# wwyuan2023/VITS

Hardware: AMD Instinct MI355X
Metric: 22.05 kHz audio samples/sec/GPU (infer RTF) + train utt/sec at 1/2/4/8 MI355X (higher is better)
Workload: dtype fp32; 1 GPU; SynthesizerTrn.infer_p2 batch=16 Tx=100 Ty=500 (configs/base.json, 16 kHz, hop 192) per GPU; global_batch=16, seq_len=500, parallelism=single GPU, graph=False

## Files before the change

### vits_amd/csrc/resblock_f32p.hip

```cpp
#include <type_traits>

#include "conv1d_impl.h"

namespace {

using vits_conv::fast_sigmoid;
using vits_conv::fast_tanh;
using vits_conv::split3_bf16x4;

constexpr int RP_GROUP = 3;
struct RpGroup {
  vits_resblock_pair_desc d[RP_GROUP];
  int n;
  int batch;
  int bn;
};

typedef __bf16 bf16x8 __attribute__((ext_vector_type(8)));
typedef __bf16 bf16x4 __attribute__((ext_vector_type(4)));
typedef __bf16 bf16x2 __attribute__((ext_vector_type(2)));
typedef float f32x4v __attribute__((ext_vector_type(4)));

template <int MODE>
struct RpT {
  typedef float xt;
  typedef __bf16 lt;
  static constexpr int NPL = 3;
};
template <>
struct RpT<1> {
  typedef __bf16 xt;
  typedef __bf16 lt;
  static constexpr int NPL = 1;
};
template <>
struct RpT<2> {
  typedef _Float16 xt;
  typedef _Float16 lt;
  static constexpr int NPL = 1;
};
__host__ __device__ constexpr int rp_npl(int mode) { return mode == 0 ? 3 : 1; }

__host__ __device__ constexpr int rp_ng(int C) { return C <= 64 ? 256 : 128; }
#ifndef VITS_RP_TM64
#define VITS_RP_TM64 1
#endif
#ifndef VITS_RP_TM128
#define VITS_RP_TM128 1
#endif
#ifndef VITS_RP_TM256
#define VITS_RP_TM256 1
#endif
#ifdef VITS_RP_OTHER_SIDE
#define VITS_RP_SIDE(tm) (3 - (tm))
#else
#define VITS_RP_SIDE(tm) (tm)
#endif
__host__ __device__ constexpr int rp_tm(int C, int mode = 0) {
  return C == 32     ? 1
         : mode != 0 ? 2
         : C == 64   ? VITS_RP_SIDE(VITS_RP_TM64)
         : C == 128  ? VITS_RP_SIDE(VITS_RP_TM128)
                     : VITS_RP_SIDE(VITS_RP_TM256);
}
__host__ __device__ constexpr int rp_threads(int C, int tm) {
  return (C / (32 * tm)) * (rp_ng(C) / 64) * 64;
}
#ifndef VITS_RP_KC32
#define VITS_RP_KC32 32
#endif
__host__ __device__ constexpr int rp_kc(int C, int mode = 0) {
  return C == 256 ? 64 : C == 32 ? VITS_RP_KC32 : 16;
}
__host__ __device__ inline int rp_xcols(int NG, int k, int dil) {
  return ((NG + (k - 1) * dil + 3 + 3) >> 2) << 2;
}
__host__ __device__ inline int rp_lds_bytes(int C, int k, int dil, int mode = 0) {
  const int NG = rp_ng(C), npl = rp_npl(mode);
  const int nbuf = rp_kc(C, mode) < C ? 2 : 1;
  const int xs = nbuf * npl * rp_xcols(NG, k, dil) * (rp_kc(C, mode) + 4);
  const int gsz = npl * (NG + 16) * (C / 2 + 8);
  return 4 * 2 * C + 2 * (xs > gsz ? xs : gsz) + 64;
}
__host__ __device__ constexpr int rp_occ(int C, int, int tm) {
  return tm == 1 && C >= 64 ? 4 : C == 256 ? 1 : 2;
}

__device__ __forceinline__ float rp_gate(float a, float b) {
#pragma clang fp contract(off)
  return fast_tanh(a) * fast_sigmoid(b);
}

__device__ __forceinline__ float rp_max(float a, float b) {
  float r;
  asm("v_max_f32 %0, %1, %2" : "=v"(r) : "v"(a), "v"(b));
  return r;
}

template <typename T>
__device__ __forceinline__ T rp_fresh(T v) {
  asm volatile("" : "+v"(v));
  return v;
}

template <typename T>
__device__ __forceinline__ const T* rp_sbase(const T* p) {
  uint64_t u = reinterpret_cast<uint64_t>(p);
  asm("" : "+s"(u));
  return (const T*)reinterpret_cast<const __attribute__((address_space(1))) T*>(u);
}

template <int C, int MODE = 0, bool MEAN = false, int TM = rp_tm(C, MODE)>
__global__ __launch_bounds__(rp_threads(C, TM), rp_occ(C, MODE, TM)) void resblock_f32p_kernel(
    const RpGroup G) {
  typedef std::integral_constant<bool, true> edge_t;
  typedef std::integral_constant<bool, false> interior_t;
  typedef typename RpT<MODE>::xt xt;
  typedef typename RpT<MODE>::lt lt;
  constexpr int NPL = RpT<MODE>::NPL;
  typedef lt lt8 __attribute__((ext_vector_type(8)));
  typedef lt lt4 __attribute__((ext_vector_type(4)));
  typedef lt lt2 __attribute__((ext_vector_type(2)));
  typedef xt xt4 __attribute__((ext_vector_type(4)));
  constexpr int H = C / 2;
  static_assert(TM == 1 || (TM == 2 && C >= 64), "wave tile rows");
  constexpr int NT = rp_threads(C, TM);
  constexpr int WAVES_M = C / (32 * TM);
  constexpr int WAVES_N = NT / 64 / WAVES_M;
  constexpr int NG = 64 * WAVES_N;
  static_assert(NG == rp_ng(C), "tile columns");
  constexpr int TN = 2;
  constexpr int KC = rp_kc(C, MODE);
  constexpr int KCP = KC + 4;
  constexpr int GP = H + 8;
  constexpr int GPL = (NG + 16) * GP;
  constexpr int S1 = C / 16, S2 = H / 16;
  constexpr int NU = ((KC / 4) * ((NG + 102) / 4) + NT - 1) / NT;
  typedef lt8 av_t;
  constexpr int NB = NPL == 3 ? TN : 1;
  constexpr bool REMAT = TM == 1 && C >= 64;

  const int gi = MEAN ? 0 : (int)blockIdx.z / G.batch;
  const int b = (int)blockIdx.z - gi * G.batch;
  const int Tn = G.d[gi].t_len;
  const int L = G.d[gi].lengths ? min(Tn, (int)G.d[gi].lengths[b]) : Tn;
  const int BN = MEAN ? G.bn : NG - (G.d[gi].k - 1);
  const int n0 = blockIdx.x * BN;
  if (n0 >= Tn) return;
  if (G.d[gi].lengths && G.d[gi].len_skip > 0 && n0 >= L + G.d[gi].len_skip) return;

  extern __shared__ float smem[];
  float* const erow = smem;
  lt* const reg = reinterpret_cast<lt*>(smem + 2 * C);

  const int tid = threadIdx.x;
  const int lane = tid & 63;
  const int wid = __builtin_amdgcn_readfirstlane(tid >> 6);
  const int wn = (wid % WAVES_N) * 64;
  const int wm = (wid / WAVES_N) * (32 * TM);
  const int l32 = lane & 31;
  const int lhi = lane >> 5;

  float msum[TM][TN][MEAN ? 16 : 1];

#pragma unroll 1
  for (int br = 0; br < (MEAN ? G.n : 1); ++br) {
    const vits_resblock_pair_desc& p = G.d[MEAN ? br : gi];
    const int k = p.k;
    const int dil = p.dil;
    const int p1 = (k - 1) * dil / 2;
    const int p2 = (k - 1) / 2;
    const int tw0 = n0 - p2 - p1;
    const int xstart = tw0 & ~3;
    const int xcols = rp_xcols(NG, k, dil);
    const bool interior = xstart >= 0 && xstart + xcols <= Tn && n0 - p2 + NG <= L;
    if (MEAN && br > 0) __syncthreads();

    {
      const float* cond = p.cond ? p.cond + (int64_t)b * p.cond_bstride : nullptr;
      for (int r = tid; r < 2 * C; r += NT) {
        float e = 0.f;
        if (r < C) {
          const int idx = (r & 1) ? H + (r >> 1) : (r >> 1);
          if (p.b1) e = p.b1[idx];
          if (cond) e += cond[idx];
        } else if (p.b2) {
          e = p.b2[r - C];
        }
        erow[r] = e;
      }
    }

    f32x16 acc[TM][TN];
#pragma unroll
    for (int i = 0; i < TM; ++i)
#pragma unroll
      for (int j = 0; j < TN; ++j)
#pragma unroll
        for (int r = 0; r < 16; ++r) acc[i][j][r] = 0.f;

    auto mma = [&](av_t (*a)[TM], const av_t* bh, const av_t* bm, const av_t* bl) {
#pragma unroll
      for (int mi = 0; mi < TM; ++mi)
#pragma unroll
        for (int ni = 0; ni < TN; ++ni) {
          f32x16 c = acc[mi][ni];
          if constexpr (MODE == 0) {
            c = __builtin_amdgcn_mfma_f32_32x32x16_bf16(a[0][mi], bl[ni], c, 0, 0, 0);
            c = __builtin_amdgcn_mfma_f32_32x32x16_bf16(a[2][mi], bh[ni], c, 0, 0, 0);
            c = __builtin_amdgcn_mfma_f32_32x32x16_bf16(a[1][mi], bm[ni], c, 0, 0, 0);
            c = __builtin_amdgcn_mfma_f32_32x32x16_bf16(a[0][mi], bm[ni], c, 0, 0, 0);
            c = __builtin_amdgcn_mfma_f32_32x32x16_bf16(a[1][mi], bh[ni], c, 0, 0, 0);
            c = __builtin_amdgcn_mfma_f32_32x32x16_bf16(a[0][mi], bh[ni], c, 0, 0, 0);
          } else if constexpr (MODE == 1) {
            c = __builtin_amdgcn_mfma_f32_32x32x16_bf16(a[0][mi], bh[ni], c, 0, 0, 0);
          } else {
            c = __builtin_amdgcn_mfma_f32_32x32x16_f16(a[0][mi], bh[ni], c, 0, 0, 0);
          }
          acc[mi][ni] = c;
        }
    };
    auto loadA = [&](const lt* w, uint32_t al, int64_t wstep, int m_pad, int s, int total,
                     av_t (*a)[TM]) {
      const lt* wp = w + (int64_t)(s < total ? s : total - 1) * wstep + (int64_t)wm * 8;
      const uint32_t av = REMAT ? rp_fresh(al) : al;
#pragma unroll
      for (int q = 0; q < NPL; ++q)
#pragma unroll
        for (int mi = 0; mi < TM; ++mi)
          if constexpr (REMAT)
            a[q][mi] = *reinterpret_cast<const av_t*>(
                reinterpret_cast<const char*>(rp_sbase(wp + ((int64_t)q * m_pad + mi * 32) * 8)) +
                av);
          else
            a[q][mi] = *reinterpret_cast<const av_t*>(
                reinterpret_cast<const char*>(wp + ((int64_t)q * m_pad + mi * 32) * 8) + av);
    };

    av_t a0[NPL][TM], a1[NPL][TM];
    av_t bh0[TN], bm0[NB], bl0[NB], bh1[TN], bm1[NB], bl1[NB];

    const xt* xb = reinterpret_cast<const xt*>(p.x) + (int64_t)b * p.x_bstride;
    {
      const int xsh = tw0 - xstart;
      const int nunits = (KC / 4) * (xcols >> 2);
      const int xpl = xcols * KCP;
      lt* const xbuf0 = reg;
      lt* const xbuf1 = reg + NPL * xpl;
      const float slope = p.in_slope;
      constexpr bool XB = KC * sizeof(xt) <= 2 * C;
      constexpr uint32_t XU = XB ? (uint32_t)sizeof(xt) : 1u;
      xt4 xr[NU][4];
      uint32_t xoff[NU];
      bool xok[NU];
#pragma unroll
      for (int q = 0; q < NU; ++q) {
        const int u = tid + NT * q;
        const int tt = xstart + 4 * (u / (KC / 4));
        xok[q] = u < nunits && tt >= 0 && tt < Tn;
        xoff[q] = xok[q] ? (uint32_t)(4 * (u % (KC / 4)) * p.x_cstride + tt) * XU : 0;
      }
      auto gload = [&](int ch) __attribute__((always_inline)) {
        const xt* base = xb + (int64_t)ch * KC * p.x_cstride;
#pragma unroll
        for (int q = 0; q < NU; ++q) {
          if (q * NT < nunits) {
            const uint32_t xo = REMAT ? rp_fresh(xoff[q]) : xoff[q];
#pragma unroll
            for (int i = 0; i < 4; ++i) {
              const xt* row = base + (int64_t)i * p.x_cstride;
              if constexpr (REMAT) row = rp_sbase(row);
              xr[q][i] = *reinterpret_cast<const xt4*>(reinterpret_cast<const char*>(row) +
                                                       (size_t)xo * (sizeof(xt) / XU));
            }
          }
        }
      };
      const bool xfast = interior && slope > 0.f && slope < 1.f;
      auto lstore_as = [&](lt* xs, auto edge) __attribute__((always_inline)) {
        const int ftid = REMAT ? rp_fresh(tid) : tid;
#pragma unroll
        for (int q = 0; q < NU; ++q) {
          const int u = ftid + NT * q;
          if (q * NT < nunits && u < nunits) {
            f32x4v v[4];
#pragma unroll
            for (int i = 0; i < 4; ++i)
#pragma unroll
              for (int e = 0; e < 4; ++e) {
                float t = (float)xr[q][i][e];
                if constexpr (decltype(edge)::value) {
                  t = t < 0.f ? t * slope : t;
                  v[i][e] = xok[q] ? t : 0.f;
                } else {
                  v[i][e] = rp_max(t, t * slope);
                }
              }
            lt* xh = xs + 4 * (u / (KC / 4)) * KCP + 4 * (u % (KC / 4));
#pragma unroll
            for (int e = 0; e < 4; ++e) {
              const f32x4v w = {v[0][e], v[1][e], v[2][e], v[3][e]};
              if constexpr (NPL == 3) {
                bf16x4 h4, m4, l4;
                split3_bf16x4(w, h4, m4, l4);
                *reinterpret_cast<bf16x4*>(xh + e * KCP) = h4;
                *reinterpret_cast<bf16x4*>(xh + xpl + e * KCP) = m4;
                *reinterpret_cast<bf16x4*>(xh + 2 * xpl + e * KCP) = l4;
              } else {
                lt4 w4;
#pragma unroll
                for (int i = 0; i < 4; ++i) w4[i] = (lt)w[i];
                *reinterpret_cast<lt4*>(xh + e * KCP) = w4;
              }
            }
          }
        }
      };
      auto lstore = [&](lt* xs) __attribute__((always_inline)) {
        if (xfast)
          lstore_as(xs, interior_t());
        else
          lstore_as(xs, edge_t());
      };
      auto loadB = [&](const lt* xs, int j, int g, av_t* bh, av_t* bm, av_t* bl) {
        const int P4 = xpl / 4;
#pragma unroll
        for (int ni = 0; ni < TN; ++ni) {
          const lt4* xp = reinterpret_cast<const lt4*>(
              xs + (wn + ni * 32 + l32 + j * dil + xsh) * KCP + 16 * g + 8 * lhi);
          bh[ni] = __builtin_shufflevector(xp[0], xp[1], 0, 1, 2, 3, 4, 5, 6, 7);
          if constexpr (NPL == 3) {
            bm[ni] = __builtin_shufflevector(xp[P4], xp[P4 + 1], 0, 1, 2, 3, 4, 5, 6, 7);
            bl[ni] = __builtin_shufflevector(xp[2 * P4], xp[2 * P4 + 1], 0, 1, 2, 3, 4, 5, 6, 7);
          }
        }
      };
      const lt* wl = reinterpret_cast<const lt*>(p.w1);
      const uint32_t al = (uint32_t)((lhi * NPL) * p.m_pad1 + l32) * (uint32_t)(8 * sizeof(lt));
      const int64_t wstep = (int64_t)16 * NPL * p.m_pad1;
      const int total = S1 * k;
      const int nst = (KC / 16) * k;
      loadA(wl, al, wstep, p.m_pad1, 0, total, a0);
      gload(0);
      lstore(xbuf0);
      __syncthreads();
      for (int ch = 0; ch < C / KC; ++ch) {
        const bool more = ch + 1 < C / KC;
        if (more) gload(ch + 1);
        const lt* xs = (ch & 1) ? xbuf1 : xbuf0;
        const int s0 = ch * nst;
        int j = 0, g = 0;
        auto next = [&]() {
          if (++j == k) {
            j = 0;
            ++g;
          }
        };
        loadB(xs, 0, 0, bh0, bm0, bl0);
        int st = 0;
        for (; st + 2 <= nst; st += 2) {
          next();
          loadA(wl, al, wstep, p.m_pad1, s0 + st + 1, total, a1);
          loadB(xs, j, g, bh1, bm1, bl1);
          __builtin_amdgcn_sched_barrier(0);
          mma(a0, bh0, bm0, bl0);
          __builtin_amdgcn_sched_barrier(0);
          next();
          loadA(wl, al, wstep, p.m_pad1, s0 + st + 2, total, a0);
          if (st + 2 < nst) loadB(xs, j, g, bh0, bm0, bl0);
          __builtin_amdgcn_sched_barrier(0);
          mma(a1, bh1, bm1, bl1);
          __builtin_amdgcn_sched_barrier(0);
        }
        if (st < nst) {
          loadA(wl, al, wstep, p.m_pad1, s0 + nst, total, a1);
          __builtin_amdgcn_sched_barrier(0);
          mma(a0, bh0, bm0, bl0);
#pragma unroll
          for (int q = 0; q < NPL; ++q)
#pragma unroll
            for (int mi = 0; mi < TM; ++mi) a0[q][mi] = a1[q][mi];
        }
        if (more) lstore((ch & 1) ? xbuf0 : xbuf1);
        __syncthreads();
      }
    }

    lt* const gs = reg;
    auto gate = [&](auto edge) __attribute__((always_inline)) {
      const int flane = REMAT ? rp_fresh(lane) : lane;
      const int l32 = flane & 31, lhi = flane >> 5;
#pragma unroll
      for (int mi = 0; mi < TM; ++mi) {
        f32x4v er[4];
#pragma unroll
        for (int g = 0; g < 4; ++g)
          er[g] = *reinterpret_cast<const f32x4v*>(erow + wm + mi * 32 + 4 * lhi + 8 * g);
#pragma unroll
        for (int ni = 0; ni < TN; ++ni) {
          const int col = wn + ni * 32 + l32;
          const int t = n0 - p2 + col;
          const bool in = t >= 0 && t < L;
#pragma unroll
          for (int r = 0; r < 16; r += 4) {
            const int row = wm + mi * 32 + 4 * lhi + 8 * (r >> 2);
            const f32x4v e = er[r >> 2];
            float g0 = rp_gate(acc[mi][ni][r] + e[0], acc[mi][ni][r + 1] + e[1]);
            float g1 = rp_gate(acc[mi][ni][r + 2] + e[2], acc[mi][ni][r + 3] + e[3]);
            if constexpr (decltype(edge)::value) {
              g0 = in ? g0 : 0.f;
              g1 = in ? g1 : 0.f;
            }
            lt* gp = gs + col * GP + (row >> 1);
            if constexpr (NPL == 3) {
              const f32x4v w = {g0, g1, 0.f, 0.f};
              bf16x4 h4, m4, l4;
              split3_bf16x4(w, h4, m4, l4);
              *reinterpret_cast<bf16x2*>(gp) = __builtin_shufflevector(h4, h4, 0, 1);
              *reinterpret_cast<bf16x2*>(gp + GPL) = __builtin_shufflevector(m4, m4, 0, 1);
              *reinterpret_cast<bf16x2*>(gp + 2 * GPL) = __builtin_shufflevector(l4, l4, 0, 1);
            } else {
              lt2 v2;
              v2[0] = (lt)g0;
              v2[1] = (lt)g1;
              *reinterpret_cast<lt2*>(gp) = v2;
            }
          }
#pragma unroll
          for (int r = 0; r < 16; ++r) acc[mi][ni][r] = 0.f;
        }
      }
    };
    if (interior)
      gate(interior_t());
    else
      gate(edge_t());
    for (int i = tid; i < NPL * 16 * H; i += NT) {
      const int pl = i / (16 * H);
      const int e = i - pl * 16 * H;
      gs[pl * GPL + (NG + e / H) * GP + e % H] = (lt)0.f;
    }
    __syncthreads();

    {
      const int flane = REMAT ? rp_fresh(lane) : lane;
      const int l32 = flane & 31, lhi = flane >> 5;
      const lt* wl = reinterpret_cast<const lt*>(p.w2);
      const uint32_t al = (uint32_t)((lhi * NPL) * p.m_pad2 + l32) * (uint32_t)(8 * sizeof(lt));
      const int64_t wstep = (int64_t)16 * NPL * p.m_pad2;
      const int total = S2 * k;
      const lt* gl = gs + (wn + l32) * GP + 8 * lhi;
      int j = 0, g = 0;
      auto loadB = [&](av_t* bh, av_t* bm, av_t* bl) {
        const lt* x = gl + j * GP + 16 * g;
#pragma unroll
        for (int ni = 0; ni < TN; ++ni) {
          bh[ni] = *reinterpret_cast<const av_t*>(x + ni * 32 * GP);
          if constexpr (NPL == 3) {
            bm[ni] = *reinterpret_cast<const av_t*>(x + ni * 32 * GP + GPL);
            bl[ni] = *reinterpret_cast<const av_t*>(x + ni * 32 * GP + 2 * GPL);
          }
        }
        if (++j == k) {
          j = 0;
          ++g;
        }
      };
      loadA(wl, al, wstep, p.m_pad2, 0, total, a0);
      loadB(bh0, bm0, bl0);
      int s = 0;
      for (; s + 2 <= total; s += 2) {
        loadA(wl, al, wstep, p.m_pad2, s + 1, total, a1);
        loadB(bh1, bm1, bl1);
        __builtin_amdgcn_sched_barrier(0);
        mma(a0, bh0, bm0, bl0);
        __builtin_amdgcn_sched_barrier(0);
        loadA(wl, al, wstep, p.m_pad2, s + 2, total, a0);
        if (s + 2 < total) loadB(bh0, bm0, bl0);
        __builtin_amdgcn_sched_barrier(0);
        mma(a1, bh1, bm1, bl1);
        __builtin_amdgcn_sched_barrier(0);
      }
      if (s < total) mma(a0, bh0, bm0, bl0);
    }

    xt* const yb = reinterpret_cast<xt*>(p.y) + (int64_t)b * p.y_bstride;
    const bool accum = !MEAN && p.accumulate;
    const float div = MEAN ? (float)G.n : p.post_div;
    const bool last = !MEAN || br == G.n - 1;
    auto epilogue = [&](auto edge) __attribute__((always_inline)) {
      const int flane = REMAT ? rp_fresh(lane) : lane;
      const int l32 = flane & 31, lhi = flane >> 5;
#pragma unroll
      for (int mi = 0; mi < TM; ++mi) {
        const xt* const xrow = xb + (int64_t)(wm + mi * 32) * p.x_cstride;
        xt* const yrow = yb + (int64_t)(wm + mi * 32) * p.y_cstride;
        f32x4v e2[4];
#pragma unroll
        for (int g = 0; g < 4; ++g)
          e2[g] = *reinterpret_cast<const f32x4v*>(erow + C + wm + mi * 32 + 4 * lhi + 8 * g);
#pragma unroll
        for (int ni = 0; ni < TN; ++ni) {
          const int col = wn + ni * 32 + l32;
          const int t = n0 + col;
          const bool st = decltype(edge)::value ? col < BN && t < Tn : col < BN;
          const int tc = st ? t : 0;
          const uint32_t xv = (uint32_t)(4 * lhi * p.x_cstride + tc) * (uint32_t)sizeof(xt);
          const uint32_t yv = (uint32_t)(4 * lhi * p.y_cstride + tc) * (uint32_t)sizeof(xt);
          auto xat = [&](int r) __attribute__((always_inline)) -> const xt& {
            const xt* row = xrow + (int64_t)((r & 3) + 8 * (r >> 2)) * p.x_cstride;
            return *reinterpret_cast<const xt*>(reinterpret_cast<const char*>(row) + xv);
          };
          auto yat = [&](int r) __attribute__((always_inline)) -> xt& {
            xt* row = yrow + (int64_t)((r & 3) + 8 * (r >> 2)) * p.y_cstride;
            return *reinterpret_cast<xt*>(reinterpret_cast<char*>(row) + yv);
          };
          float o[16];
#pragma unroll
          for (int r = 0; r < 16; ++r) {
            const float rv = (float)xat(r);
            const float v = acc[mi][ni][r] + e2[r >> 2][r & 3];
            o[r] = rv + v;
          }
          if constexpr (MEAN) {
#pragma unroll
            for (int r = 0; r < 16; ++r) {
              o[r] = br == 0 ? o[r] : msum[mi][ni][r] + o[r];
              msum[mi][ni][r] = o[r];
            }
          }
          if (accum) {
#pragma unroll
            for (int r = 0; r < 16; ++r)
              o[r] = (float)yat(r) + o[r];
          }
          if (last) {
            if (div != 1.0f) {
#pragma unroll
              for (int r = 0; r < 16; ++r) o[r] = o[r] / div;
            }
            if (st) {
#pragma unroll
              for (int r = 0; r < 16; ++r) {
                if constexpr (decltype(edge)::value) o[r] = t < L ? o[r] : 0.f;
                yat(r) = (xt)o[r];
              }
            }
          }
        }
      }
    };
    if (interior)
      epilogue(interior_t());
    else
      epilogue(edge_t());
  }
}

template <int C, int MODE = 0, bool MEAN = false, int TM = rp_tm(C, MODE)>
int rp_launch(const RpGroup& g, hipStream_t s) {
  int lds = 0, gx = 0;
  for (int i = 0; i < g.n; ++i) {
    const vits_resblock_pair_desc& d = g.d[i];
    const int l = rp_lds_bytes(C, d.k, d.dil, MODE);
    if (l > lds) lds = l;
    const int BN = MEAN ? g.bn : rp_ng(C) - (d.k - 1);
    const int x = (d.t_len + BN - 1) / BN;
    if (x > gx) gx = x;
  }
  if (lds > 160 * 1024) return VITS_E_UNSUP;
  hipLaunchKernelGGL((resblock_f32p_kernel<C, MODE, MEAN, TM>),
                     dim3(gx, 1, MEAN ? g.batch : g.n * g.batch), dim3(rp_threads(C, TM)), lds, s,
                     g);
  return vits_launch_status();
}

int rp_check(const vits_resblock_pair_desc& d, int mode = 0) {
  VITS_CHECK_ARG(d.x && d.w1 && d.w2 && d.y);
  VITS_CHECK_ARG(reinterpret_cast<const void*>(d.y) != reinterpret_cast<const void*>(d.x));
  VITS_CHECK_SHAPE(d.channels == 32 || d.channels == 64 || d.channels == 128 ||
                   d.channels == 256);
  VITS_CHECK_SHAPE(d.k >= 1 && d.k <= 15 && (d.k & 1) == 1 && d.dil >= 1 && d.t_len > 0);
  VITS_CHECK_SHAPE((d.k - 1) * d.dil <= 96);
  VITS_CHECK_SHAPE(d.m_pad1 >= d.channels && d.m_pad2 >= d.channels && (d.m_pad1 & 3) == 0 &&
                   (d.m_pad2 & 3) == 0);
  VITS_CHECK_SHAPE(d.cin_pad1 >= d.channels && d.cin_pad2 >= d.channels / 2);
  VITS_CHECK_SHAPE((d.t_len & 3) == 0 && (d.x_cstride & 3) == 0 && (d.x_bstride & 3) == 0 &&
                   d.x_cstride >= d.t_len && d.y_cstride >= d.t_len &&
                   (reinterpret_cast<uintptr_t>(d.x) & (mode ? 7 : 15)) == 0);
  VITS_CHECK_SHAPE((int64_t)d.channels * d.x_cstride < (1LL << 31));
  VITS_CHECK_SHAPE((int64_t)d.channels * d.y_cstride < (1LL << 31));
  VITS_CHECK_SHAPE((reinterpret_cast<uintptr_t>(d.w1) & 15) == 0 &&
                   (reinterpret_cast<uintptr_t>(d.w2) & 15) == 0);
  return VITS_OK;
}

}

int vits_rp16_256(const vits_resblock_pair_desc* d, int n, int batch, int wdtype,
                  hipStream_t s) {
  if (!d || n < 1 || n > RP_GROUP || batch < 1) return VITS_E_ARG;
  if (wdtype != VITS_WDT_BF16 && wdtype != VITS_WDT_F16) return VITS_E_ARG;
  const int mode = wdtype == VITS_WDT_BF16 ? 1 : 2;
  RpGroup g;
  g.n = n;
  g.batch = batch;
  g.bn = 0;
  for (int i = 0; i < n; ++i) {
    const int rc = rp_check(d[i], mode);
    if (rc) return rc;
    if (d[i].channels != d[0].channels) return VITS_E_SHAPE;
    g.d[i] = d[i];
  }
  if (d[0].channels != 256) return VITS_E_SHAPE;
  return mode == 1 ? rp_launch<256, 1>(g, s) : rp_launch<256, 2>(g, s);
}

extern "C" int vits_resblock_pair_f32p_forward(const vits_resblock_pair_desc* d, int n, int batch,
                                               void* stream) {
  if (!d || n < 1 || n > RP_GROUP || batch < 1) return VITS_E_ARG;
  RpGroup g;
  g.n = n;
  g.batch = batch;
  g.bn = 0;
  for (int i = 0; i < n; ++i) {
    const int rc = rp_check(d[i]);
    if (rc) return rc;
    if (d[i].channels != d[0].channels) return VITS_E_SHAPE;
    g.d[i] = d[i];
  }
  hipStream_t s = as_stream(stream);
  int rc;
  if (d[0].channels == 32)
    rc = rp_launch<32>(g, s);
  else if (d[0].channels == 64)
    rc = rp_launch<64>(g, s);
  else if (d[0].channels == 128)
    rc = rp_launch<128>(g, s);
  else
    rc = rp_launch<256>(g, s);
  return count_ok(rc, VITS_CNT_RESBLOCK);
}

extern "C" int vits_resblock_pair_f32p_mean_forward(const vits_resblock_pair_desc* d, int n,
                                                    int batch, void* stream) {
  if (!d || n < 1 || n > RP_GROUP || batch < 1) return VITS_E_ARG;
  RpGroup g;
  g.n = n;
  g.batch = batch;
  int kmax = 1;
  for (int i = 0; i < n; ++i) {
    const int rc = rp_check(d[i]);
    if (rc) return rc;
    VITS_CHECK_SHAPE(d[i].channels == 32);
    VITS_CHECK_SHAPE(d[i].t_len == d[0].t_len && d[i].lengths == d[0].lengths &&
                     d[i].len_skip == d[0].len_skip && d[i].y == d[0].y &&
                     d[i].y_bstride == d[0].y_bstride && d[i].y_cstride == d[0].y_cstride);
    VITS_CHECK_ARG(reinterpret_cast<const void*>(d[0].y) != reinterpret_cast<const void*>(d[i].x));
    if (d[i].k > kmax) kmax = d[i].k;
    g.d[i] = d[i];
  }
  g.bn = rp_ng(32) - (kmax - 1);
  return count_ok(rp_launch<32, 0, true>(g, as_stream(stream)), VITS_CNT_RESBLOCK);
}
```

Before: 80.28 million output samples/s.

## Use single-buffered KC=16 chunks for C=32 resblocks to raise occupancy

For the 32-channel resblock, the input channel chunk drops from 32 to 16 and the LDS staging becomes a single buffer, with an extra barrier before each refill. The prefetch is split around the MMA step, offsets are recomputed instead of kept in registers, and launch bounds move to occupancy 4. In MEAN mode the running branch sum is kept in the output buffer rather than in registers by default. The aim is lower register and LDS use so more waves fit per CU, at the cost of extra syncs and extra output reads and writes.

New measurement: 80.26 million output samples/s, median of 3. No clear change (-0.0%).

```diff
diff --git a/vits_amd/csrc/resblock_f32p.hip b/vits_amd/csrc/resblock_f32p.hip
--- a/vits_amd/csrc/resblock_f32p.hip
+++ b/vits_amd/csrc/resblock_f32p.hip
@@ -67,23 +67,42 @@
   return (C / (32 * tm)) * (rp_ng(C) / 64) * 64;
 }
 #ifndef VITS_RP_KC32
-#define VITS_RP_KC32 32
+#define VITS_RP_KC32 16
 #endif
-__host__ __device__ constexpr int rp_kc(int C, int mode = 0) {
-  return C == 256 ? 64 : C == 32 ? VITS_RP_KC32 : 16;
+#ifndef VITS_RP_MEAN_REGS
+#define VITS_RP_MEAN_REGS 0
+#endif
+static_assert(VITS_RP_KC32 == 16 || VITS_RP_KC32 == 32, "VITS_RP_KC32");
+static_assert(VITS_RP_MEAN_REGS == 0 || VITS_RP_MEAN_REGS == 1, "VITS_RP_MEAN_REGS");
+#ifdef VITS_RP_OTHER_SIDE
+constexpr int RP_KC32 = 48 - VITS_RP_KC32;
+constexpr bool RP_MEAN_REGS = !VITS_RP_MEAN_REGS;
+#else
+constexpr int RP_KC32 = VITS_RP_KC32;
+constexpr bool RP_MEAN_REGS = VITS_RP_MEAN_REGS;
+#endif
+__host__ __device__ constexpr int rp_kc(int C, int mode = 0, bool mean = false) {
+  return C == 256 ? 64 : C == 32 ? (mean && RP_MEAN_REGS ? 32 : RP_KC32) : 16;
+}
+__host__ __device__ constexpr int rp_nbuf(int C, int mode = 0, bool mean = false) {
+  return rp_kc(C, mode, mean) < C && C != 32 ? 2 : 1;
 }
 __host__ __device__ inline int rp_xcols(int NG, int k, int dil) {
   return ((NG + (k - 1) * dil + 3 + 3) >> 2) << 2;
 }
-__host__ __device__ inline int rp_lds_bytes(int C, int k, int dil, int mode = 0) {
+__host__ __device__ inline int rp_lds_bytes(int C, int k, int dil, int mode = 0,
+                                            bool mean = false) {
   const int NG = rp_ng(C), npl = rp_npl(mode);
-  const int nbuf = rp_kc(C, mode) < C ? 2 : 1;
-  const int xs = nbuf * npl * rp_xcols(NG, k, dil) * (rp_kc(C, mode) + 4);
+  const int nbuf = rp_nbuf(C, mode, mean);
+  const int xs = nbuf * npl * rp_xcols(NG, k, dil) * (rp_kc(C, mode, mean) + 4);
   const int gsz = npl * (NG + 16) * (C / 2 + 8);
   return 4 * 2 * C + 2 * (xs > gsz ? xs : gsz) + 64;
 }
-__host__ __device__ constexpr int rp_occ(int C, int, int tm) {
-  return tm == 1 && C >= 64 ? 4 : C == 256 ? 1 : 2;
+__host__ __device__ constexpr int rp_occ(int C, int mode, int tm, bool mean = false) {
+  return C == 32 ? (rp_kc(C, mode, mean) < C ? 4 : 2)
+         : tm == 1 && C >= 64 ? 4
+         : C == 256           ? 1
+                              : 2;
 }
 
 __device__ __forceinline__ float rp_gate(float a, float b) {
@@ -111,7 +130,8 @@
 }
 
 template <int C, int MODE = 0, bool MEAN = false, int TM = rp_tm(C, MODE)>
-__global__ __launch_bounds__(rp_threads(C, TM), rp_occ(C, MODE, TM)) void resblock_f32p_kernel(
+__global__ __launch_bounds__(rp_threads(C, TM),
+                             rp_occ(C, MODE, TM, MEAN)) void resblock_f32p_kernel(
     const RpGroup G) {
   typedef std::integral_constant<bool, true> edge_t;
   typedef std::integral_constant<bool, false> interior_t;
@@ -130,7 +150,7 @@
   constexpr int NG = 64 * WAVES_N;
   static_assert(NG == rp_ng(C), "tile columns");
   constexpr int TN = 2;
-  constexpr int KC = rp_kc(C, MODE);
+  constexpr int KC = rp_kc(C, MODE, MEAN);
   constexpr int KCP = KC + 4;
   constexpr int GP = H + 8;
   constexpr int GPL = (NG + 16) * GP;
@@ -138,7 +158,10 @@
   constexpr int NU = ((KC / 4) * ((NG + 102) / 4) + NT - 1) / NT;
   typedef lt8 av_t;
   constexpr int NB = NPL == 3 ? TN : 1;
-  constexpr bool REMAT = TM == 1 && C >= 64;
+  constexpr bool REMAT = rp_occ(C, MODE, TM, MEAN) == 4;
+  constexpr bool XSINGLE = KC < C && rp_nbuf(C, MODE, MEAN) == 1;
+  constexpr bool MSUM = MEAN && RP_MEAN_REGS;
+  constexpr int CHUNROLL = XSINGLE ? 2 : 1;
 
   const int gi = MEAN ? 0 : (int)blockIdx.z / G.batch;
   const int b = (int)blockIdx.z - gi * G.batch;
@@ -153,19 +176,23 @@
   float* const erow = smem;
   lt* const reg = reinterpret_cast<lt*>(smem + 2 * C);
 
-  const int tid = threadIdx.x;
-  const int lane = tid & 63;
-  const int wid = __builtin_amdgcn_readfirstlane(tid >> 6);
+  const int tid0 = threadIdx.x;
+  const int lane0 = tid0 & 63;
+  const int wid = __builtin_amdgcn_readfirstlane(tid0 >> 6);
   const int wn = (wid % WAVES_N) * 64;
   const int wm = (wid / WAVES_N) * (32 * TM);
-  const int l32 = lane & 31;
-  const int lhi = lane >> 5;
-
-  float msum[TM][TN][MEAN ? 16 : 1];
+  const int l320 = lane0 & 31;
+  const int lhi0 = lane0 >> 5;
+
+  float msum[TM][TN][MSUM ? 16 : 1];
 
 #pragma unroll 1
   for (int br = 0; br < (MEAN ? G.n : 1); ++br) {
     const vits_resblock_pair_desc& p = G.d[MEAN ? br : gi];
+    const int tid = MEAN && REMAT ? rp_fresh(tid0) : tid0;
+    const int lane = MEAN && REMAT ? tid & 63 : lane0;
+    const int l32 = MEAN && REMAT ? lane & 31 : l320;
+    const int lhi = MEAN && REMAT ? lane >> 5 : lhi0;
     const int k = p.k;
     const int dil = p.dil;
     const int p1 = (k - 1) * dil / 2;
@@ -250,22 +277,32 @@
       const float slope = p.in_slope;
       constexpr bool XB = KC * sizeof(xt) <= 2 * C;
       constexpr uint32_t XU = XB ? (uint32_t)sizeof(xt) : 1u;
+      constexpr int NUMIN = XSINGLE ? (KC / 4) * ((NG + 4) / 4) : 0;
       xt4 xr[NU][4];
-      uint32_t xoff[NU];
-      bool xok[NU];
-#pragma unroll
-      for (int q = 0; q < NU; ++q) {
-        const int u = tid + NT * q;
+      auto xunit = [&](int t, int q, bool& ok) __attribute__((always_inline)) -> uint32_t {
+        const int u = t + NT * q;
         const int tt = xstart + 4 * (u / (KC / 4));
-        xok[q] = u < nunits && tt >= 0 && tt < Tn;
-        xoff[q] = xok[q] ? (uint32_t)(4 * (u % (KC / 4)) * p.x_cstride + tt) * XU : 0;
+        ok = u < nunits && tt >= 0 && tt < Tn;
+        return ok ? (uint32_t)(4 * (u % (KC / 4)) * p.x_cstride + tt) * XU : 0;
+      };
+      uint32_t xoff[XSINGLE ? 1 : NU];
+      bool xok[XSINGLE ? 1 : NU];
+      if constexpr (!XSINGLE) {
+#pragma unroll
+        for (int q = 0; q < NU; ++q) xoff[q] = xunit(tid, q, xok[q]);
       }
-      auto gload = [&](int ch) __attribute__((always_inline)) {
+      auto gload = [&](int ch, int q0, int q1) __attribute__((always_inline)) {
         const xt* base = xb + (int64_t)ch * KC * p.x_cstride;
 #pragma unroll
         for (int q = 0; q < NU; ++q) {
-          if (q * NT < nunits) {
-            const uint32_t xo = REMAT ? rp_fresh(xoff[q]) : xoff[q];
+          if (q >= q0 && q < q1 && (q * NT < NUMIN || q * NT < nunits)) {
+            uint32_t xo;
+            if constexpr (XSINGLE) {
+              bool ok;
+              xo = xunit(rp_fresh(tid), q, ok);
+            } else {
+              xo = REMAT ? rp_fresh(xoff[q]) : xoff[q];
+            }
 #pragma unroll
             for (int i = 0; i < 4; ++i) {
               const xt* row = base + (int64_t)i * p.x_cstride;
@@ -283,6 +320,13 @@
         for (int q = 0; q < NU; ++q) {
           const int u = ftid + NT * q;
           if (q * NT < nunits && u < nunits) {
+            bool ok = true;
+            if constexpr (decltype(edge)::value) {
+              if constexpr (XSINGLE)
+                xunit(ftid, q, ok);
+              else
+                ok = xok[q];
+            }
             f32x4v v[4];
 #pragma unroll
             for (int i = 0; i < 4; ++i)
@@ -291,7 +335,7 @@
                 float t = (float)xr[q][i][e];
                 if constexpr (decltype(edge)::value) {
                   t = t < 0.f ? t * slope : t;
-                  v[i][e] = xok[q] ? t : 0.f;
+                  v[i][e] = ok ? t : 0.f;
                 } else {
                   v[i][e] = rp_max(t, t * slope);
                 }
@@ -326,8 +370,15 @@
         const int P4 = xpl / 4;
 #pragma unroll
         for (int ni = 0; ni < TN; ++ni) {
-          const lt4* xp = reinterpret_cast<const lt4*>(
-              xs + (wn + ni * 32 + l32 + j * dil + xsh) * KCP + 16 * g + 8 * lhi);
+          const lt4* xp;
+          if constexpr (XSINGLE) {
+            const int fl = rp_fresh(lane);
+            xp = reinterpret_cast<const lt4*>(
+                xs + (wn + ni * 32 + (fl & 31) + j * dil + xsh) * KCP + 16 * g + 8 * (fl >> 5));
+          } else {
+            xp = reinterpret_cast<const lt4*>(
+                xs + (wn + ni * 32 + l32 + j * dil + xsh) * KCP + 16 * g + 8 * lhi);
+          }
           bh[ni] = __builtin_shufflevector(xp[0], xp[1], 0, 1, 2, 3, 4, 5, 6, 7);
           if constexpr (NPL == 3) {
             bm[ni] = __builtin_shufflevector(xp[P4], xp[P4 + 1], 0, 1, 2, 3, 4, 5, 6, 7);
@@ -341,13 +392,14 @@
       const int total = S1 * k;
       const int nst = (KC / 16) * k;
       loadA(wl, al, wstep, p.m_pad1, 0, total, a0);
-      gload(0);
+      gload(0, 0, NU);
       lstore(xbuf0);
       __syncthreads();
+#pragma unroll CHUNROLL
       for (int ch = 0; ch < C / KC; ++ch) {
         const bool more = ch + 1 < C / KC;
-        if (more) gload(ch + 1);
-        const lt* xs = (ch & 1) ? xbuf1 : xbuf0;
+        if (more) gload(ch + 1, 0, XSINGLE ? 1 : NU);
+        const lt* xs = !XSINGLE && (ch & 1) ? xbuf1 : xbuf0;
         const int s0 = ch * nst;
         int j = 0, g = 0;
         auto next = [&]() {
@@ -374,14 +426,26 @@
         }
         if (st < nst) {
           loadA(wl, al, wstep, p.m_pad1, s0 + nst, total, a1);
+          if constexpr (XSINGLE) {
+            if (more) gload(ch + 1, 1, NU);
+          }
           __builtin_amdgcn_sched_barrier(0);
           mma(a0, bh0, bm0, bl0);
 #pragma unroll
           for (int q = 0; q < NPL; ++q)
 #pragma unroll
             for (int mi = 0; mi < TM; ++mi) a0[q][mi] = a1[q][mi];
-        }
-        if (more) lstore((ch & 1) ? xbuf0 : xbuf1);
+        } else if constexpr (XSINGLE) {
+          if (more) gload(ch + 1, 1, NU);
+        }
+        if constexpr (XSINGLE) {
+          if (more) {
+            __syncthreads();
+            lstore(xbuf0);
+          }
+        } else {
+          if (more) lstore((ch & 1) ? xbuf0 : xbuf1);
+        }
         __syncthreads();
       }
     }
@@ -485,7 +549,7 @@
     }
 
     xt* const yb = reinterpret_cast<xt*>(p.y) + (int64_t)b * p.y_bstride;
-    const bool accum = !MEAN && p.accumulate;
+    const bool accum = MEAN ? !MSUM && br > 0 : (bool)p.accumulate;
     const float div = MEAN ? (float)G.n : p.post_div;
     const bool last = !MEAN || br == G.n - 1;
     auto epilogue = [&](auto edge) __attribute__((always_inline)) {
@@ -522,7 +586,7 @@
             const float v = acc[mi][ni][r] + e2[r >> 2][r & 3];
             o[r] = rv + v;
           }
-          if constexpr (MEAN) {
+          if constexpr (MSUM) {
 #pragma unroll
             for (int r = 0; r < 16; ++r) {
               o[r] = br == 0 ? o[r] : msum[mi][ni][r] + o[r];
@@ -534,17 +598,15 @@
             for (int r = 0; r < 16; ++r)
               o[r] = (float)yat(r) + o[r];
           }
-          if (last) {
-            if (div != 1.0f) {
-#pragma unroll
-              for (int r = 0; r < 16; ++r) o[r] = o[r] / div;
-            }
-            if (st) {
-#pragma unroll
-              for (int r = 0; r < 16; ++r) {
-                if constexpr (decltype(edge)::value) o[r] = t < L ? o[r] : 0.f;
-                yat(r) = (xt)o[r];
-              }
+          if (last && div != 1.0f) {
+#pragma unroll
+            for (int r = 0; r < 16; ++r) o[r] = o[r] / div;
+          }
+          if ((last || !MSUM) && st) {
+#pragma unroll
+            for (int r = 0; r < 16; ++r) {
+              if constexpr (decltype(edge)::value) o[r] = t < L ? o[r] : 0.f;
+              yat(r) = (xt)o[r];
             }
           }
         }
@@ -562,7 +624,7 @@
   int lds = 0, gx = 0;
   for (int i = 0; i < g.n; ++i) {
     const vits_resblock_pair_desc& d = g.d[i];
-    const int l = rp_lds_bytes(C, d.k, d.dil, MODE);
+    const int l = rp_lds_bytes(C, d.k, d.dil, MODE, MEAN);
     if (l > lds) lds = l;
     const int BN = MEAN ? g.bn : rp_ng(C) - (d.k - 1);
     const int x = (d.t_len + BN - 1) / BN;
```
